# malani86/unet-DC-segmentation

Measured on AMD Instinct MI355X. Metric: images/sec fwd+bwd, 512x512x1 U-Net-DC, bs=8/GPU, higher is better.
Workload: dtype bf16

## Files before the change

### unet_dc_segmentation_amd/build.py

```python
from __future__ import annotations

import os
import shutil
import subprocess
import sys

HERE = os.path.dirname(os.path.abspath(__file__))
CSRC = os.path.join(HERE, "csrc")
SOURCES = ["abi.hip", "igemm_conv.hip", "igemm_dma.hip", "igemm_dma16.hip", "igemm_halo.hip", "igemm_lattice.hip", "wgrad.hip", "wgrad_dma.hip", "wgrad_fused.hip", "wgrad_rect.hip", "convt_wgrad.hip", "first_conv.hip", "first_conv_mfma.hip", "elementwise.hip", "loss.hip", "optim.hip", "ccl.hip", "preprocess.hip", "augment.hip", "density.hip"]
HEADERS = ["common.h", "kernels.h", "lds_dma.h", "wgrad_frag.h", "igemm_epilogue.h", "igemm_epilogue16.h", os.path.join("..", "..", "include", "unetdc_hip.h")]
OUT = os.path.join(HERE, "libunetdc_hip.so")


def _hipcc():
    for cand in (shutil.which("hipcc"), "/opt/rocm/bin/hipcc"):
        if cand and os.path.exists(cand):
            return cand
    raise RuntimeError("hipcc not found (ROCm toolchain required to build the gfx950 kernels)")


def needs_build():
    if not os.path.exists(OUT):
        return True
    t = os.path.getmtime(OUT)
    deps = [os.path.join(CSRC, f) for f in SOURCES + HEADERS]
    return any(os.path.getmtime(d) > t for d in deps)


FLAGS = ["--offload-arch=gfx950", "-O3", "-std=c++17", "-fPIC", "-Wall", "-Wno-unused-function", "-fno-slp-vectorize"]
OBJ_DIR = os.path.join(CSRC, "_obj")


def _includes(path, seen=None):
    import re
    seen = set() if seen is None else seen
    for m in re.finditer(r'^\s*#include\s+"([^"]+)"', open(path).read(), re.M):
        q = os.path.normpath(os.path.join(os.path.dirname(path), m.group(1)))
        if q not in seen and os.path.exists(q):
            seen.add(q)
            _includes(q, seen)
    return seen


def _object_key(src):
    import hashlib
    h = hashlib.sha256(" ".join(FLAGS).encode())
    for q in [src] + sorted(_includes(src)):
        h.update(open(q, "rb").read())
    return h.hexdigest()[:16]


def build(force=False, verbose=True):
    if not force and not needs_build():
        return OUT
    from concurrent.futures import ThreadPoolExecutor
    os.makedirs(OBJ_DIR, exist_ok=True)
    hipcc = _hipcc()

    def one(f):
        src = os.path.join(CSRC, f)
        obj = os.path.join(OBJ_DIR, f"{os.path.splitext(f)[0]}.{_object_key(src)}.o")
        if force or not os.path.exists(obj):
            for old in os.listdir(OBJ_DIR):
                if old.startswith(os.path.splitext(f)[0] + "."):
                    os.unlink(os.path.join(OBJ_DIR, old))
            cmd = [hipcc, *FLAGS, "-c", src, "-o", obj]
            if verbose:
                print("[unetdc build]", " ".join(cmd), flush=True)
            r = subprocess.run(cmd, capture_output=True, text=True)
            if r.returncode != 0:
                sys.stderr.write(r.stdout + r.stderr)
                raise RuntimeError(f"hipcc failed on {f}")
        return obj

    with ThreadPoolExecutor(max_workers=min(8, os.cpu_count() or 1)) as ex:
        objs = list(ex.map(one, SOURCES))
    cmd = [hipcc, "--offload-arch=gfx950", "-shared", "-fPIC", *objs, "-o", OUT]
    r = subprocess.run(cmd, capture_output=True, text=True)
    if r.returncode != 0:
        sys.stderr.write(r.stdout + r.stderr)
        raise RuntimeError("hipcc failed linking libunetdc_hip.so")
    return OUT


def _objdump():
    for cand in (shutil.which("llvm-objdump"), "/opt/rocm/lib/llvm/bin/llvm-objdump"):
        if cand and os.path.exists(cand):
            return cand
    raise RuntimeError("llvm-objdump not found")


def device_code_objects(so_path=OUT):
    import struct
    data = open(so_path, "rb").read()
    magic, pos, out = b"__CLANG_OFFLOAD_BUNDLE__", 0, []
    while True:
        i = data.find(magic, pos)
        if i < 0:
            return out
        n, = struct.unpack_from("<Q", data, i + 24)
        q = i + 32
        for _ in range(n):
            off, size, idl = struct.unpack_from("<QQQ", data, q)
            q += 24
            tid = data[q:q + idl].decode()
            q += idl
            if "gfx950" in tid and size:
                out.append(data[i + off:i + off + size])
        pos = i + 24


def packed_f32_report(so_path=OUT):
    import re
    import tempfile
    rep = {}
    for k, elf in enumerate(device_code_objects(so_path)):
        with tempfile.NamedTemporaryFile(suffix=".co") as f:
            f.write(elf)
            f.flush()
            r = subprocess.run([_objdump(), "-d", "--no-show-raw-insn", f.name], capture_output=True, text=True)
        if r.returncode != 0:
            raise RuntimeError("llvm-objdump failed: " + r.stderr[:300])
        cur = None
        for line in r.stdout.splitlines():
            m = re.match(r"^[0-9a-f]+ <(\S+)>:", line)
            if m:
                cur = m.group(1)
                rep.setdefault(cur, 0)
            elif cur and re.search(r"\bv_pk_(add|mul|fma)_f32\b", line):
                rep[cur] += 1
    return rep


if __name__ == "__main__":
    build(force="--force" in sys.argv)
```

### unet_dc_segmentation_amd/csrc/igemm_conv.hip

```cpp
#include <stdlib.h>

#include <stdio.h>

#include "kernels.h"

namespace unetdc {

template <typename T> struct Mma;
template <> struct Mma<bf16_t> {
  __device__ static __forceinline__ void run(f32x16& acc, const u32x4& a, const u32x4& b) {
    acc = __builtin_amdgcn_mfma_f32_32x32x16_bf16(__builtin_bit_cast(bf16x8, a), __builtin_bit_cast(bf16x8, b),
                                                  acc, 0, 0, 0);
  }
};
template <> struct Mma<float> {
  __device__ static __forceinline__ void run(f32x16& acc, const u32x4& a, const u32x4& b) {
#pragma unroll
    for (int s = 0; s < 4; ++s) {
      const unsigned int ua = a[s], ub = b[s];
      acc = __builtin_amdgcn_mfma_f32_32x32x2f32(bits_f32(ua), bits_f32(ub), acc, 0, 0, 0);
    }
  }
};

template <typename T> __device__ __forceinline__ void store_pair(T* dst, float v0, float v1);
template <> __device__ __forceinline__ void store_pair<float>(float* dst, float v0, float v1) {
  *reinterpret_cast<float2*>(dst) = make_float2(v0, v1);
}
template <> __device__ __forceinline__ void store_pair<bf16_t>(bf16_t* dst, float v0, float v1) {
  bf16_t lo = (bf16_t)v0, hi = (bf16_t)v1;
  *reinterpret_cast<unsigned int*>(dst) = (unsigned int)__builtin_bit_cast(unsigned short, lo) |
                                          ((unsigned int)__builtin_bit_cast(unsigned short, hi) << 16);
}

template <typename T, int WM, int WN>
__global__ __launch_bounds__(256, 2) void igemm_conv_kernel(const IgemmParams p) {
  constexpr int BM = 64 * WM, BN = 64 * WN;
  constexpr int AI = BM / 32, BI = BN / 32;
  constexpr int KE = 128 / (int)sizeof(T);
  constexpr int EPC = 16 / (int)sizeof(T);
  constexpr int STAGE = (BM + BN) * 128;
  extern __shared__ __attribute__((aligned(16))) unsigned char smem[];

  const int tid = threadIdx.x, lane = tid & 63, wave = tid >> 6;
  const int wm = wave / WN, wn = wave % WN;
  const int tile = xcd_remap(blockIdx.x, gridDim.x);
  const int mblk = tile / p.nblocks, nblk = tile - mblk * p.nblocks;
  const int m0 = mblk * BM, n0 = nblk * BN;
  const int c = tid & 7, r0 = tid >> 3;
  const T* __restrict__ xg = reinterpret_cast<const T*>(p.x);
  const T* __restrict__ wg = reinterpret_cast<const T*>(p.w);

  int pix[AI], ys[AI], xs[AI];
  unsigned tapmask = 0;
  const int HoWo = p.Ho * p.Wo;
#pragma unroll
  for (int i = 0; i < AI; ++i) {
    const int m = m0 + r0 + 32 * i;
    if (m < p.M) {
      const int n = m / HoWo, rem = m - n * HoWo;
      const int oy = rem / p.Wo, ox = rem - oy * p.Wo;
      ys[i] = oy * p.stride;
      xs[i] = ox * p.stride;
      pix[i] = (n * p.Hi + ys[i]) * p.Wi + xs[i];
    } else {
      ys[i] = -(1 << 28);
      xs[i] = 0;
      pix[i] = 0;
    }
    for (int t = 0; t < p.ntaps; ++t) {
      const int iy = ys[i] + p.offy[t], ix = xs[i] + p.offx[t];
      if ((unsigned)iy < (unsigned)p.Hi && (unsigned)ix < (unsigned)p.Wi) tapmask |= 1u << t;
    }
  }
  {
    unsigned* sm_u = reinterpret_cast<unsigned*>(smem);
    if (tid == 0) sm_u[0] = 0;
    __syncthreads();
    if (tapmask) atomicOr(&sm_u[0], tapmask);
    __syncthreads();
    tapmask = sm_u[0];
    __syncthreads();
  }
  const int nkc = p.Cin / KE;
  const int nsteps = __popc(tapmask) * nkc;

  const int swz_w = (r0 >> 1) & 7;
  int a_wr[AI], b_wr[BI];
#pragma unroll
  for (int i = 0; i < AI; ++i) a_wr[i] = (r0 + 32 * i) * 128 + ((c ^ swz_w) << 4);
#pragma unroll
  for (int i = 0; i < BI; ++i) {
    const int row = r0 + 32 * i, grp = row >> 6, cc = row & 63;
    const int lrow = grp * 64 + (cc & 1) * 32 + (cc >> 1);
    b_wr[i] = BM * 128 + lrow * 128 + ((c ^ ((lrow >> 1) & 7)) << 4);
  }
  const int r = lane & 31, h = lane >> 5;
  const int swz_r = (r >> 1) & 7;
  int a_rd[2][4], b_rd[2][4];
#pragma unroll
  for (int t2 = 0; t2 < 2; ++t2)
#pragma unroll
    for (int g = 0; g < 4; ++g) {
      const int ch = ((2 * g + h) ^ swz_r) << 4;
      a_rd[t2][g] = (wm * 64 + t2 * 32 + r) * 128 + ch;
      b_rd[t2][g] = BM * 128 + (wn * 64 + t2 * 32 + r) * 128 + ch;
    }

  f32x16 acc[2][2];
#pragma unroll
  for (int i = 0; i < 2; ++i)
#pragma unroll
    for (int j = 0; j < 2; ++j)
#pragma unroll
      for (int e = 0; e < 16; ++e) acc[i][j][e] = 0.f;

  u32x4 ra[AI], rb[BI];
  int lt = 0, lkc = 0;
  while (lt < p.ntaps && !((tapmask >> lt) & 1u)) ++lt;

  auto gload = [&]() {
    const int dy = p.offy[lt], dx = p.offx[lt];
    const int dpix = dy * p.Wi + dx;
    const int koff = lkc * KE + c * EPC;
#pragma unroll
    for (int i = 0; i < AI; ++i) {
      const int iy = ys[i] + dy, ix = xs[i] + dx;
      const bool ok = (unsigned)iy < (unsigned)p.Hi && (unsigned)ix < (unsigned)p.Wi;
      u32x4 v = {0u, 0u, 0u, 0u};
      if (ok) v = ld16(xg + ((long)(pix[i] + dpix) * p.ldx + koff));
      ra[i] = v;
    }
#pragma unroll
    for (int i = 0; i < BI; ++i)
      rb[i] = ld16(wg + ((long)(lt * p.Cout + n0 + r0 + 32 * i) * p.Cin + koff));
    if (++lkc == nkc) {
      lkc = 0;
      do { ++lt; } while (lt < p.ntaps && !((tapmask >> lt) & 1u));
    }
  };
  auto lds_store = [&](int stage) {
    unsigned char* base = smem + stage * STAGE;
#pragma unroll
    for (int i = 0; i < AI; ++i) st16(base + a_wr[i], ra[i]);
#pragma unroll
    for (int i = 0; i < BI; ++i) st16(base + b_wr[i], rb[i]);
  };

  if (nsteps > 0) {
    gload();
    lds_store(0);
  }
  __syncthreads();
  for (int s = 0; s < nsteps; ++s) {
    const bool more = (s + 1 < nsteps);
    if (more) gload();
    const unsigned char* base = smem + (s & 1) * STAGE;
#pragma unroll
    for (int g = 0; g < 4; ++g) {
      const u32x4 a0 = ld16(base + a_rd[0][g]), a1 = ld16(base + a_rd[1][g]);
      const u32x4 b0 = ld16(base + b_rd[0][g]), b1 = ld16(base + b_rd[1][g]);
      Mma<T>::run(acc[0][0], a0, b0);
      Mma<T>::run(acc[0][1], a0, b1);
      Mma<T>::run(acc[1][0], a1, b0);
      Mma<T>::run(acc[1][1], a1, b1);
    }
    if (more) lds_store((s + 1) & 1);
    __syncthreads();
  }

  const int col = n0 + wn * 64 + 2 * r;
  T* __restrict__ og = reinterpret_cast<T*>(p.out);
  float k0a = 0.f, k0b = 0.f, k1a = 0.f, k1b = 0.f;
  int shuf_ab = 0, shuf_co = col;
  if (p.mode == MODE_AFFINE_RELU) {
    k0a = p.scale[col]; k0b = p.scale[col + 1];
    k1a = p.shift[col]; k1b = p.shift[col + 1];
  } else if (p.mode == MODE_SHUFFLE) {
    shuf_ab = col / p.shuf_c;
    shuf_co = col - shuf_ab * p.shuf_c;
    if (p.bias) { k1a = p.bias[shuf_co]; k1b = p.bias[shuf_co + 1]; }
  } else if (p.bias) {
    k1a = p.bias[col]; k1b = p.bias[col + 1];
  }
  float s0 = 0.f, q0 = 0.f, s1 = 0.f, q1 = 0.f;
#pragma unroll
  for (int mi = 0; mi < 2; ++mi) {
#pragma unroll
    for (int reg = 0; reg < 16; ++reg) {
      const int m = m0 + wm * 64 + mi * 32 + (reg & 3) + 8 * (reg >> 2) + 4 * h;
      if (m >= p.M) continue;
      float v0 = acc[mi][0][reg], v1 = acc[mi][1][reg];
      if (p.mode == MODE_AFFINE_RELU) {
        v0 = fmaxf(fmaf(v0, k0a, k1a), 0.f);
        v1 = fmaxf(fmaf(v1, k0b, k1b), 0.f);
        store_pair<T>(og + (long)m * p.ldo + col, v0, v1);
      } else if (p.mode == MODE_SHUFFLE) {
        v0 += k1a; v1 += k1b;
        const int n = m / HoWo, rem = m - n * HoWo;
        const int oy = rem / p.Wo, ox = rem - oy * p.Wo;
        const long dst = ((long)(n * 2 * p.Ho + 2 * oy + (shuf_ab >> 1)) * (2 * p.Wo) + 2 * ox + (shuf_ab & 1));
        store_pair<T>(og + dst * p.ldo + shuf_co, v0, v1);
      } else {
        v0 += k1a; v1 += k1b;
        store_pair<T>(og + (long)m * p.ldo + col, v0, v1);
        if (p.mode == MODE_STATS) {
          const float t0 = round_through<T>(v0), t1 = round_through<T>(v1);
          s0 += t0; q0 = fmaf(t0, t0, q0);
          s1 += t1; q1 = fmaf(t1, t1, q1);
        }
      }
    }
  }
  if (p.mode == MODE_STATS) {
    s0 += __shfl_xor(s0, 32, 64); q0 += __shfl_xor(q0, 32, 64);
    s1 += __shfl_xor(s1, 32, 64); q1 += __shfl_xor(q1, 32, 64);
    float* red = reinterpret_cast<float*>(smem);
    if (h == 0) {
      red[(wave * 4 + 0) * 32 + r] = s0;
      red[(wave * 4 + 1) * 32 + r] = q0;
      red[(wave * 4 + 2) * 32 + r] = s1;
      red[(wave * 4 + 3) * 32 + r] = q1;
    }
    __syncthreads();
    if (tid < BN) {
      const int wn2 = tid >> 6, c2 = tid & 63, r2 = c2 >> 1, e = c2 & 1;
      float su = 0.f, sq = 0.f;
#pragma unroll
      for (int w2 = 0; w2 < WM; ++w2) {
        su += red[((w2 * WN + wn2) * 4 + e * 2 + 0) * 32 + r2];
        sq += red[((w2 * WN + wn2) * 4 + e * 2 + 1) * 32 + r2];
      }
      p.stats[((long)mblk * 2 + 0) * p.Cout + n0 + tid] = su;
      p.stats[((long)mblk * 2 + 1) * p.Cout + n0 + tid] = sq;
    }
  }
}

int igemm_mblocks(long M, int Cout) { (void)Cout; return ceil_div(M, 256); }

template <typename T, int WM, int WN>
static int launch_cfg(IgemmParams& p, hipStream_t stream) {
  constexpr int BM = 64 * WM, BN = 64 * WN;
  constexpr int LDS = 2 * (BM + BN) * 128;
  if (const int rc_ = ensure_dynamic_lds(reinterpret_cast<const void*>(&igemm_conv_kernel<T, WM, WN>), LDS, "igemm_conv_kernel")) return rc_;
  p.mblocks = ceil_div(p.M, BM);
  p.nblocks = p.Cout / BN;
  const long nwg = (long)p.mblocks * p.nblocks;
  hipLaunchKernelGGL((igemm_conv_kernel<T, WM, WN>), dim3((unsigned)nwg), dim3(256), LDS, stream, p);
  char nm[96];
  snprintf(nm, sizeof(nm), "igemm_conv_kernel<%s, %d, %d>", sizeof(T) == 2 ? "__bf16" : "float", WM, WN);
  note_kernel(nm);
  return check_launch("igemm_conv_kernel");
}

IgemmPlan plan_igemm(const IgemmParams& p, int dtype) {
  IgemmPlan pl{};
  const bool lattice = igemm_lattice_supported(p, dtype);
  if (p.in_scale) {
    if (lattice && p.mode == MODE_STATS && (p.Cout % 128 == 0 || p.Cin <= 256)) {
      pl.route = IGEMM_LATTICE;
      pl.writes_act = p.Cout % 128 == 0 && (long)p.M * p.Cin * 2 < (1L << 32);
    }
    return pl;
  }
  if (lattice) {
    pl.route = IGEMM_LATTICE;
    return pl;
  }
  if (igemm_halo_supported(p, dtype)) {
    pl.route = IGEMM_HALO;
    return pl;
  }
  const long es = dtype == UNETDC_BF16 ? 2 : 4;
  const long HoWo = (long)p.Ho * p.Wo;
  const long xbytes = (p.M / HoWo) * p.Hi * p.Wi * p.ldx * es;
  const long wbytes = (long)p.ntaps * p.Cout * p.Cin * es;
  const long opix = p.mode == MODE_SHUFFLE ? 4L * p.M : (long)p.M;
  const long obytes = opix * p.ldo * es, ybytes = p.mode == MODE_BNBWD ? (long)p.M * p.bn_ldy * es : 0;
  if (!(xbytes < (1L << 31) && wbytes < (1L << 31) && obytes < (1L << 32) && ybytes < (1L << 32) && p.M % HoWo == 0)) {
    pl.route = IGEMM_FIRSTGEN;
    pl.cfg = (p.Cout % 128 == 0) && p.mode != MODE_STATS;
    return pl;
  }
  const long blocks_a = (long)((p.M + 255) / 256) * (p.Cout / 256);
  const bool use_a = p.Cout % 256 == 0 && p.M >= 256 * 64 && blocks_a >= 200;
  const bool use_b = !use_a && p.Cout % 128 == 0;
  pl.route = IGEMM_DMA;
  pl.cfg = use_a ? 1 : (use_b ? 2 : 3);
  if (dtype == UNETDC_BF16 && p.M % 16 == 0 && !(p.mode == MODE_SHUFFLE && p.Wo % 16 != 0)) {
    pl.route = IGEMM_DMA16;
    const long blocks_b = (long)((p.M + 255) / 256) * (p.Cout / 128);
    if (pl.cfg == 2 && p.mode == MODE_SHUFFLE && p.Cout % 256 == 0 && blocks_a >= 200) pl.cfg = 1;
    else if (pl.cfg == 2 && blocks_b >= 100 && blocks_b < 200) pl.cfg = 3;
  }
  return pl;
}

int launch_igemm(IgemmParams& p, int dtype, hipStream_t stream) {
  const int esz = dtype == UNETDC_BF16 ? 2 : 4;
  const int ke = 128 / esz;
  UNETDC_REQUIRE(dtype == UNETDC_F32 || dtype == UNETDC_BF16, "igemm: bad dtype %d", dtype);
  UNETDC_REQUIRE(p.x && p.w && p.out, "igemm: null tensor pointer");
  UNETDC_REQUIRE(p.M > 0 && p.Cin > 0 && p.Cout > 0, "igemm: empty problem");
  UNETDC_REQUIRE(p.Cin % ke == 0, "igemm: Cin=%d must be a multiple of %d for this dtype", p.Cin, ke);
  UNETDC_REQUIRE(p.Cout % 64 == 0, "igemm: Cout=%d must be a multiple of 64", p.Cout);
  UNETDC_REQUIRE(p.ldx % (16 / esz) == 0 && p.ldo % (16 / esz) == 0, "igemm: ld not 16-byte aligned");
  UNETDC_REQUIRE(((uintptr_t)p.x % 16 == 0) && ((uintptr_t)p.w % 16 == 0) && ((uintptr_t)p.out % 16 == 0),
                 "igemm: pointers must be 16-byte aligned");
  UNETDC_REQUIRE(p.ntaps >= 1 && p.ntaps <= 9, "igemm: ntaps out of range");
  UNETDC_REQUIRE((long)p.M < (1L << 31) - 512, "igemm: too many pixels");
  if (p.mode == MODE_SHUFFLE) UNETDC_REQUIRE(p.shuf_c % 64 == 0, "igemm: convT channels must be a multiple of 64");
  if (p.mode == MODE_STATS) UNETDC_REQUIRE(p.stats != nullptr, "igemm: stats buffer missing");
  if (p.mode == MODE_AFFINE_RELU) UNETDC_REQUIRE(p.scale && p.shift, "igemm: scale/shift missing");
  if (p.mode == MODE_BNBWD)
    UNETDC_REQUIRE(p.stats && p.bn_y && p.scale && p.shift && p.bn_mean && p.bn_rstd, "igemm: BN-backward inputs missing");
  {
    const long howo = (long)p.Ho * p.Wo;
    const bool p2 = (p.Wo & (p.Wo - 1)) == 0 && (howo & (howo - 1)) == 0;
    p.wo_shift = p2 ? __builtin_ctz((unsigned)p.Wo) : -1;
    p.howo_shift = p2 ? __builtin_ctzl((unsigned long)howo) : -1;
  }
  const IgemmPlan pl = plan_igemm(p, dtype);
  switch (pl.route) {
    case IGEMM_LATTICE: return launch_igemm_lattice(p, stream);
    case IGEMM_HALO: return launch_igemm_halo(p, dtype, stream);
    case IGEMM_DMA: return launch_igemm_dma(p, pl.cfg, dtype, stream);
    case IGEMM_DMA16: return launch_igemm_dma16(p, pl.cfg, stream);
    case IGEMM_FIRSTGEN:
      if (p.mode == MODE_BNBWD) {
        set_error("igemm: the first-generation kernel has no fused BatchNorm-backward sums");
        return UNETDC_EUNSUPPORTED;
      }
      if (dtype == UNETDC_BF16) return pl.cfg ? launch_cfg<bf16_t, 2, 2>(p, stream) : launch_cfg<bf16_t, 4, 1>(p, stream);
      return pl.cfg ? launch_cfg<float, 2, 2>(p, stream) : launch_cfg<float, 4, 1>(p, stream);
  }
  set_error("igemm: input normalisation asked for a shape / configuration the lattice kernel does not take");
  return UNETDC_EUNSUPPORTED;
}

}
```

### unet_dc_segmentation_amd/csrc/kernels.h

```cpp
#pragma once
#include "common.h"
#include "../../include/unetdc_hip.h"

namespace unetdc {

enum { MODE_STORE = 0, MODE_STATS = 1, MODE_AFFINE_RELU = 2, MODE_SHUFFLE = 3, MODE_BNBWD = 4 };
#define UNETDC_EUNSUPPORTED (-4)

struct IgemmParams {
  const void* x;
  const void* w;
  void* out;
  const float* bias;
  const float* scale;
  const float* shift;
  float* stats;
  const void* bn_y;
  const float* bn_mean;
  const float* bn_rstd;
  int bn_ldy;
  int M, Ho, Wo, Hi, Wi, Cin, Cout, ldx, ldo, ntaps, stride, mode, shuf_c;
  int mblocks, nblocks;
  int wo_shift, howo_shift;
  int quad_bpr, quad_bpi;
  const float* in_scale;
  const float* in_shift;
  void* act_out;
  int ld_act;
  int offy[9];
  int offx[9];
};
enum IgemmRoute {
  IGEMM_UNSUPPORTED = 0,
  IGEMM_LATTICE,
  IGEMM_HALO,
  IGEMM_DMA,
  IGEMM_DMA16,
  IGEMM_FIRSTGEN,
};
struct IgemmPlan {
  int route;
  int cfg;
  bool writes_act;
};
IgemmPlan plan_igemm(const IgemmParams& p, int dtype);
int launch_igemm(IgemmParams& p, int dtype, hipStream_t stream);
int igemm_mblocks(long M, int Cout);
bool igemm_lattice_supported(const IgemmParams& p, int dtype);
bool igemm_halo_supported(const IgemmParams& p, int dtype);
int launch_igemm_lattice(IgemmParams& p, hipStream_t stream);
int launch_igemm_halo(IgemmParams& p, int dtype, hipStream_t stream);
int launch_igemm_dma(IgemmParams& p, int cfg, int dtype, hipStream_t stream);
int launch_igemm_dma16(IgemmParams& p, int cfg, hipStream_t stream);

struct WgradParams {
  const void* a;
  const void* b;
  float* part;
  int N, H, W, Hb, Wb, CI, CJ, lda, ldb, ntaps, stride;
  int P;
  int chunk;
  int ksplit, itiles, jtiles;
  int adv_y, adv_x;
  int offy[9];
  int offx[9];
  const float* in_scale;
  const float* in_shift;
};
enum WgradRoute {
  WGRAD_UNSUPPORTED = 0,
  WGRAD_CONVT,
  WGRAD_RECT,
  WGRAD_FUSED,
  WGRAD_DMA,
  WGRAD_LEGACY,
};
struct WgradPlan {
  int route;
  int ksplit;
  int chunk, tw, step;
  int steps_per_half;
  long workspace;
};
WgradPlan plan_wgrad(const WgradParams& p, int dtype);
long wgrad_workspace_bound(int N, int H, int W, int CI, int CJ, int ntaps, int dtype);
int launch_wgrad(WgradParams& p, float* out, void* workspace, long workspace_bytes, int dtype, hipStream_t stream);
bool convt_wgrad_split(int N, int H, int W, int CI, int CJ, int& ksplit, int& steps_per_half);
int launch_convt_wgrad_fused(const WgradParams& w, const WgradPlan& pl, hipStream_t stream);
int wgrad_rect_units(int N, int H, int W, int CI, int CJ, int d);
int launch_wgrad_rect(const WgradParams& w, const WgradPlan& pl, float* out, hipStream_t stream);
bool wgrad_fused_supported(int N, int H, int W, int CI, int CJ, int lda, int ldb, int d, int ntaps, int stride, int dtype);
bool wgrad_fused_bnin_supported(int d, int dtype);
long wgrad_fused_workspace_bytes(int N, int H, int W, int CI, int CJ, int dtype);
int launch_wgrad_fused(const WgradParams& w, int dtype, int* units_out, hipStream_t stream);
int wgrad_dma_tile(int CI, int CJ);
int wgrad_dma_pixel_step(int dtype, int tw);
int launch_wgrad_dma_kernel(WgradParams& p, int tw, int dtype, hipStream_t stream);

struct FirstParams {
  const float* x;
  const float* w;
  const float* bias;
  const float* scale;
  const float* shift;
  void* y;
  float* stats;
  int N, H, W, Cin, Cout, ldy, dil;
};
struct FirstWgradParams {
  const float* x;
  const void* dy;
  float* part;
  int N, H, W, Cin, Cout, lddy, dil;
  const void* bn_y; int bn_ldy;
  const float* bn_scale; const float* bn_shift; const float* bn_mean; const float* bn_rstd; const float* bn_k;
};
struct FirstPlan {
  bool mfma;
  int fwd_blocks;
  bool wgrad_mfma;
  int wgrad_blocks;
  int rows_blocks;
  long workspace;
};
FirstPlan plan_first(long P, int Cin, int Cout);
int launch_first_fwd(FirstParams& p, int dtype, hipStream_t stream);
bool first_wgrad_bn_supported(int N, int H, int W, int Cin, int Cout, int dil, int dtype);
int launch_bn_bwd_coeffs(const float* pre_parts, int pre_nparts, long count, const float* gamma, const float* rstd, float* dgamma,
                         float* dbeta, float* dbias, float* coeffs, int C, hipStream_t stream);
int first_mfma_mblocks(long P);
int first_mfma_wgrad_blocks(long P);
int launch_first_mfma_fwd(FirstParams& p, int blocks, int dtype, hipStream_t stream);
int launch_first_mfma_wgrad(FirstWgradParams& p, int blocks, int dtype, hipStream_t stream);
int launch_first_wgrad(FirstWgradParams& p, float* dw, void* workspace, long workspace_bytes, int dtype,
                       hipStream_t stream);
int launch_first_dgrad(const void* dy, int lddy, const float* w, float* dx, int N, int H, int W, int Cin, int Cout, int dil,
                       int dtype, hipStream_t stream);

struct ApplyParams {
  const void* y; void* a; void* pooled;
  const float* scale; const float* shift;
  int N, H, W, C, ldy, lda, ldp;
};
struct BnBwdParams {
  const void* dskip; const void* dpool; const void* y; void* dy;
  const float* scale; const float* shift; const float* mean; const float* rstd;
  const float* k1; const float* k2; const float* k3;
  float* parts;
  int N, H, W, C, lds, ldp, ldy, lddy;
  const float* head_dprobs; const float* head_probs; const float* head_w;
};
struct HeadParams {
  const void* a; const float* w; const float* b; float* probs;
  const float* dprobs; void* da; float* parts;
  int N, H, W, C, OC, lda, ldda;
  const void* bn_y; const float* bn_scale; const float* bn_shift; const float* bn_mean; const float* bn_rstd;
  float* bn_parts;
  int bn_ldy;
};
int launch_bn_finalize(const float* parts, int nparts, long count, const float* gamma, const float* beta, float eps,
                       float momentum, float* rm, float* rv, float* scale, float* shift, float* mean, float* rstd,
                       int C, hipStream_t stream);
int launch_bn_eval_affine(const float* gamma, const float* beta, const float* rm, const float* rv,
                          const float* conv_bias, float eps, float* scale, float* shift, int C, hipStream_t stream);
int launch_apply(ApplyParams& p, int dtype, hipStream_t stream);
long bn_bwd_workspace_bytes(int N, int H, int W, int C, int pooled, int dtype);
int launch_bn_bwd(BnBwdParams& p, const float* gamma, float* dgamma, float* dbeta, float* dbias, void* workspace,
                  long workspace_bytes, const float* pre_parts, int pre_nparts, int dtype, hipStream_t stream,
                  bool frozen = false);
int launch_bn_frozen_affine(const float* gamma, const float* beta, const float* rm, const float* rv, float eps, float* scale,
                            float* shift, float* mean, float* rstd, int C, hipStream_t stream);
int launch_stats_colsum_rows(const float* parts, int nparts, int row_floats, int c0, int c, float* out, hipStream_t stream);
int launch_bn_bwd_reduce_only(BnBwdParams& p, float* parts, long parts_floats, int* nparts, int dtype,
                              hipStream_t stream);
long head_bwd_workspace_bytes(int N, int H, int W, int C, int OC, int dtype);
int launch_head_fwd(HeadParams& p, int dtype, hipStream_t stream);
int launch_head_bwd(HeadParams& p, float* dw, float* db, void* workspace, long workspace_bytes, int dtype,
                    hipStream_t stream, int* bn_nparts = nullptr, long bn_parts_floats = 0);
int launch_pack_conv3x3(const float* w, void* wf, void* wd, int Co, int Ci, int dtype, hipStream_t stream);
int launch_pack_convT2x2(const float* w, void* wf, void* wd, int Ci, int Co, int dtype, hipStream_t stream);
int launch_pack_many(const void* table_dev, int n, long total, int dtype, hipStream_t stream);
int launch_adam_step(const void* table_dev, int n, long total_blocks, const float* flat_grad, double lr, double beta1,
                     double beta2, double eps, long step, double grad_scale, int dtype, hipStream_t stream);
int launch_stats_colsum(const float* parts, int nparts, int ctotal, int c0, int c, float* out, hipStream_t stream);
long channel_sum_workspace_bytes(long P, int C);
int launch_channel_sum(const void* x, int ldx, float* out, void* workspace, long workspace_bytes, long P, int C,
                       int dtype, hipStream_t stream);

int launch_mask_from_probs(const float* probs, int ph, int pw, float thresh, unsigned char* mask, int oh, int ow,
                           hipStream_t stream);
int launch_mask_from_probs_linear(const float* probs, int ph, int pw, float thresh, unsigned char* mask, int oh, int ow,
                                  const int* xofs, const short* xcoef, const int* yofs, const short* ycoef, hipStream_t stream);
long ccl_workspace_bytes(int h, int w);
int launch_ccl_stats(const unsigned char* mask, int h, int w, int min_area, void* workspace, long workspace_bytes,
                     int* out_count, int* out_area, long long* out_sumy, long long* out_sumx, int* out_root, int max_out,
                     hipStream_t stream);

constexpr int AUG_HFLIP = 1, AUG_VFLIP = 2, AUG_BC = 4;
constexpr int AUG_MAX_SEEDS = 64;
constexpr int AUG_MAX_BATCH = 32;
struct AugRecord {
  int src, flags, k, field;
  float alpha, beta_max;
  int reserved[2];
};
long elastic_fields_workspace_bytes(int n, int h, int w, double sigma);
int launch_elastic_fields(const unsigned* seeds, int n, int h, int w, double sigma, float alpha, float* fields,
                          void* workspace, long workspace_bytes, hipStream_t stream);
int launch_augment_gather(const float* cache_img, const unsigned char* cache_mask, int ncache, int c, int h, int w,
                          const AugRecord* params, int n, const float* fields, int nfields, float* out_img, float* out_mask,
                          hipStream_t stream);

long rolling_ball_workspace_bytes(int h, int w, int cn);
int launch_rolling_ball(const unsigned char* src, unsigned char* dst, int h, int w, int cn, int k, void* workspace,
                        long workspace_bytes, hipStream_t stream);
int launch_resize_linear_chw(const unsigned char* src, int h, int w, int cn, float* dst, int dh, int dw, const int* xofs,
                             const short* xa, const int* yofs, const short* ya, hipStream_t stream);
int launch_morph_rect(const unsigned char* src, unsigned char* dst, int h, int w, int k, bool is_max, hipStream_t stream);

long density_workspace_bytes(int h, int w);
int launch_density_maps(const unsigned char* rgb, const unsigned char* mask, int h, int w, const int* dcount, const int* darea,
                        const long long* dsumy, const long long* dsumx, int dcap, int nb_layers, double sigma,
                        const double* taps, void* workspace, long workspace_bytes, unetdc_density_stats* stats,
                        unsigned char* radial_index, unsigned char* spatial_index, unsigned char* out_blur,
                        unsigned char* out_roi, unsigned char* out_ring, float* out_radial, float* out_spatial,
                        hipStream_t stream);
int launch_density_sqrt(const long long* x, double* out, long n, hipStream_t stream);

long loss_workspace_bytes(int nimg, long hw);
int launch_loss_fwd(const float* p, const float* t, float* loss_out, float* coef, void* workspace, long workspace_bytes,
                    int nimg, long hw, float alpha, float gamma, float ratio, float smooth, hipStream_t stream);
int launch_loss_bwd(const float* p, const float* t, const float* coef, const float* gout, float* dp, int nimg, long hw,
                    float alpha, float gamma, float ratio, hipStream_t stream);

}
```

Baseline: 761.7.

## Add dedicated register-resident-weight kernel for bf16 transposed-conv forward

```diff
diff --git a/unet_dc_segmentation_amd/build.py b/unet_dc_segmentation_amd/build.py
--- a/unet_dc_segmentation_amd/build.py
+++ b/unet_dc_segmentation_amd/build.py
@@ -7,7 +7,7 @@
 
 HERE = os.path.dirname(os.path.abspath(__file__))
 CSRC = os.path.join(HERE, "csrc")
-SOURCES = ["abi.hip", "igemm_conv.hip", "igemm_dma.hip", "igemm_dma16.hip", "igemm_halo.hip", "igemm_lattice.hip", "wgrad.hip", "wgrad_dma.hip", "wgrad_fused.hip", "wgrad_rect.hip", "convt_wgrad.hip", "first_conv.hip", "first_conv_mfma.hip", "elementwise.hip", "loss.hip", "optim.hip", "ccl.hip", "preprocess.hip", "augment.hip", "density.hip"]
+SOURCES = ["abi.hip", "igemm_conv.hip", "igemm_dma.hip", "igemm_dma16.hip", "igemm_halo.hip", "igemm_lattice.hip", "wgrad.hip", "wgrad_dma.hip", "wgrad_fused.hip", "wgrad_rect.hip", "convt_wgrad.hip", "convt_fwd.hip", "first_conv.hip", "first_conv_mfma.hip", "elementwise.hip", "loss.hip", "optim.hip", "ccl.hip", "preprocess.hip", "augment.hip", "density.hip"]
 HEADERS = ["common.h", "kernels.h", "lds_dma.h", "wgrad_frag.h", "igemm_epilogue.h", "igemm_epilogue16.h", os.path.join("..", "..", "include", "unetdc_hip.h")]
 OUT = os.path.join(HERE, "libunetdc_hip.so")
 
diff --git a/unet_dc_segmentation_amd/csrc/convt_fwd.hip b/unet_dc_segmentation_amd/csrc/convt_fwd.hip
--- /dev/null
+++ b/unet_dc_segmentation_amd/csrc/convt_fwd.hip
@@ -0,0 +1,186 @@
+#include <stdio.h>
+#include <stdlib.h>
+
+#include "igemm_epilogue16.h"
+#include "kernels.h"
+#include "lds_dma.h"
+
+namespace unetdc {
+
+struct ConvtFwdParams {
+  const void* x;
+  const void* w;
+  const float* bias;
+  void* up;
+  int M, H, W, Cout, ldx, ldup;
+  int w_shift, hw_shift;
+  int mtiles, nblocks;
+};
+
+constexpr unsigned CONVT_OOB = 0x80000000u;
+
+template <int CIN> struct ConvtFwdCfg {
+  static constexpr int WGS = 2;
+  static constexpr int LDS = 2 * 64 * CIN * 2 + 256 * 4;
+};
+
+template <int CIN>
+__global__ __launch_bounds__(256, ConvtFwdCfg<CIN>::WGS) void convt_fwd_kernel(const ConvtFwdParams p) {
+#if defined(__HIP_DEVICE_COMPILE__)
+  constexpr int NKC = CIN / 64;
+  constexpr int NKG = CIN / 32;
+  constexpr int BM = 64;
+  constexpr int TMT = BM / 16;
+  constexpr int STAGE = BM * CIN * 2;
+  constexpr int PER = BM * NKC / 32;
+  constexpr int NST = TMT * 2;
+  static_assert(CIN == 128 || CIN == 256, "K");
+  static_assert(NST <= 63, "vmcnt is a 6-bit counter");
+  extern __shared__ __attribute__((aligned(16))) unsigned char smem[];
+
+  const int tid = threadIdx.x, lane = tid & 63;
+  const int wave = __builtin_amdgcn_readfirstlane(tid >> 6);
+  const int bid = xcd_remap(blockIdx.x, gridDim.x);
+  const int nblk = bid % p.nblocks;
+  const int mstride = gridDim.x / p.nblocks;
+  int mt = bid / p.nblocks;
+  if (mt >= p.mtiles) return;
+  const unsigned lds_base = lds_addr_of(smem);
+
+  const unsigned xbytes = (unsigned)p.M * (unsigned)p.ldx * 2u;
+  const unsigned obytes = (unsigned)p.M * 4u * (unsigned)p.ldup * 2u;
+  const __amdgpu_buffer_rsrc_t xr = __builtin_amdgcn_make_buffer_rsrc(const_cast<void*>(p.x), 0, xbytes, 0x00020000);
+  const __amdgpu_buffer_rsrc_t orr = __builtin_amdgcn_make_buffer_rsrc(p.up, 0, obytes, 0x00020000);
+
+  const int sub = lane >> 3, pc = lane & 7;
+  const int drow = wave * 8 + sub;
+  const unsigned dchunk = (unsigned)((pc ^ ((drow >> 1) & 7)) << 4);
+  auto issue = [&](int stage, int tile) {
+    const int m0 = tile * BM;
+    const unsigned sbase = lds_base + (unsigned)__builtin_amdgcn_readfirstlane(stage) * STAGE;
+#pragma unroll
+    for (int j = 0; j < PER; ++j) {
+      const int row = drow + 32 * (j & 1), kc = j >> 1;
+      const int m = m0 + row;
+      lds_dma16(xr, sbase + (wave + 4 * j) * 1024, m < p.M ? (unsigned)m * (unsigned)p.ldx * 2u + (unsigned)(kc * 128) + dchunk
+                                                             : CONVT_OOB, 0u);
+    }
+  };
+  issue(0, mt);
+
+  const int c16 = lane & 15, rb = lane >> 4;
+  const int nw = nblk * 256 + wave * 64;
+  const int ab = nw / p.Cout, ch = nw - ab * p.Cout + 8 * rb;
+  u32x4 wf[4][NKG];
+#pragma unroll
+  for (int j = 0; j < 4; ++j) {
+    const int col = nw + 32 * (j >> 1) + 8 * (c16 >> 2) + 4 * (j & 1) + (c16 & 3);
+    const u32x4* src = reinterpret_cast<const u32x4*>(static_cast<const bf16_t*>(p.w) + (long)col * CIN + 8 * rb);
+#pragma unroll
+    for (int g = 0; g < NKG; ++g) wf[j][g] = src[4 * g];
+  }
+  float* bias_l = reinterpret_cast<float*>(smem + 2 * STAGE);
+  bias_l[tid] = p.bias ? p.bias[(nblk * 256 + tid) % p.Cout] : 0.f;
+  const float* bias_w = bias_l + wave * 64 + 8 * rb;
+
+  const int swz = (c16 >> 1) & 7;
+  int x_rd[2];
+#pragma unroll
+  for (int h = 0; h < 2; ++h) x_rd[h] = c16 * 128 + (((4 * h + rb) ^ swz) << 4);
+  const int H2 = 2 * p.H, W2 = 2 * p.W, HW = p.H * p.W;
+  const unsigned ldob = (unsigned)p.ldup * 2u;
+
+  int cur = 0;
+  for (bool first = true;; first = false) {
+    if (first) wait_vmcnt<0>(); else wait_vmcnt<NST>();
+    raw_barrier();
+    const int next = mt + mstride;
+    const bool more = next < p.mtiles;
+    if (more) issue(cur ^ 1, next);
+
+    f32x4 acc[TMT][4];
+#pragma unroll
+    for (int i = 0; i < TMT; ++i)
+#pragma unroll
+      for (int j = 0; j < 4; ++j)
+#pragma unroll
+        for (int e = 0; e < 4; ++e) acc[i][j][e] = 0.f;
+    const unsigned char* base = smem + cur * STAGE;
+#pragma unroll
+    for (int g = 0; g < NKG; ++g)
+#pragma unroll
+      for (int i = 0; i < TMT; ++i) {
+        const u32x4 xf = ld16(base + (g >> 1) * BM * 128 + i * 16 * 128 + x_rd[g & 1]);
+#pragma unroll
+        for (int j = 0; j < 4; ++j)
+          acc[i][j] = __builtin_amdgcn_mfma_f32_16x16x32_bf16(__builtin_bit_cast(bf16x8, wf[j][g]), __builtin_bit_cast(bf16x8, xf),
+                                                              acc[i][j], 0, 0, 0);
+      }
+
+    const int m0 = mt * BM;
+#pragma unroll
+    for (int i = 0; i < TMT; ++i) {
+      const int m = m0 + 16 * i + c16;
+      int n, y, xx;
+      if (p.w_shift >= 0) {
+        n = m >> p.hw_shift;
+        const int rem = m & (HW - 1);
+        y = rem >> p.w_shift;
+        xx = rem & (p.W - 1);
+      } else {
+        n = m / HW;
+        const int rem = m - n * HW;
+        y = rem / p.W;
+        xx = rem - y * p.W;
+      }
+      const unsigned opix = (unsigned)((n * H2 + 2 * y + (ab >> 1)) * W2 + 2 * xx + (ab & 1));
+      const unsigned voff = m < p.M ? opix * ldob + (unsigned)ch * 2u : CONVT_OOB;
+#pragma unroll
+      for (int q = 0; q < 2; ++q) {
+        const f32x4 lo = acc[i][2 * q], hi = acc[i][2 * q + 1];
+        const f32x4 bl = *reinterpret_cast<const f32x4*>(bias_w + 32 * q), bh = *reinterpret_cast<const f32x4*>(bias_w + 32 * q + 4);
+        const u32x2 a = pack4_bf16(lo[0] + bl[0], lo[1] + bl[1], lo[2] + bl[2], lo[3] + bl[3]);
+        const u32x2 b = pack4_bf16(hi[0] + bh[0], hi[1] + bh[1], hi[2] + bh[2], hi[3] + bh[3]);
+        const u32x4 v = {a[0], a[1], b[0], b[1]};
+        __builtin_amdgcn_raw_buffer_store_b128(v, orr, voff, (unsigned)q * 64u, 0);
+      }
+    }
+    if (!more) break;
+    mt = next;
+    cur ^= 1;
+  }
+#endif
+}
+
+template <int CIN>
+static int launch_cfg(const ConvtFwdParams& q, hipStream_t stream) {
+  constexpr int LDS = ConvtFwdCfg<CIN>::LDS;
+  const void* fn = reinterpret_cast<const void*>(&convt_fwd_kernel<CIN>);
+  if (const int rc = ensure_dynamic_lds(fn, LDS, "convt_fwd_kernel")) return rc;
+  const long items = (long)q.mtiles * q.nblocks;
+  constexpr int FULL = 256 * ConvtFwdCfg<CIN>::WGS;
+  const long nwg = items < FULL ? items : FULL - FULL % q.nblocks;
+  hipLaunchKernelGGL((convt_fwd_kernel<CIN>), dim3((unsigned)nwg), dim3(256), LDS, stream, q);
+  note_kernel(CIN == 128 ? "convt_fwd_kernel<128>" : "convt_fwd_kernel<256>");
+  return check_launch("convt_fwd_kernel");
+}
+
+bool convt_fwd_supported(const IgemmParams& p, int dtype) {
+  if (dtype != UNETDC_BF16 || p.mode != MODE_SHUFFLE || p.ntaps != 1 || p.stride != 1) return false;
+  if (!(p.Cin == 128 || p.Cin == 256) || p.shuf_c % 64 != 0 || p.Cout != 4 * p.shuf_c || p.Cout % 256 != 0) return false;
+  return (long)p.M * p.ldx * 2 < (1L << 31) && 4L * p.M * p.ldo * 2 < (1L << 31);
+}
+
+int launch_convt_fwd(IgemmParams& p, hipStream_t stream) {
+  UNETDC_REQUIRE(convt_fwd_supported(p, UNETDC_BF16), "convt_fwd: unsupported shape");
+  ConvtFwdParams q{};
+  q.x = p.x; q.w = p.w; q.bias = p.bias; q.up = p.out;
+  q.M = p.M; q.H = p.Ho; q.W = p.Wo; q.Cout = p.shuf_c; q.ldx = p.ldx; q.ldup = p.ldo;
+  q.w_shift = p.wo_shift; q.hw_shift = p.howo_shift;
+  q.mtiles = ceil_div(p.M, 64);
+  q.nblocks = p.Cout / 256;
+  p.mblocks = q.mtiles; p.nblocks = q.nblocks;
+  return p.Cin == 128 ? launch_cfg<128>(q, stream) : launch_cfg<256>(q, stream);
+}
+
+}
diff --git a/unet_dc_segmentation_amd/csrc/igemm_conv.hip b/unet_dc_segmentation_amd/csrc/igemm_conv.hip
--- a/unet_dc_segmentation_amd/csrc/igemm_conv.hip
+++ b/unet_dc_segmentation_amd/csrc/igemm_conv.hip
@@ -293,6 +293,7 @@
     const long blocks_b = (long)((p.M + 255) / 256) * (p.Cout / 128);
     if (pl.cfg == 2 && p.mode == MODE_SHUFFLE && p.Cout % 256 == 0 && blocks_a >= 200) pl.cfg = 1;
     else if (pl.cfg == 2 && blocks_b >= 100 && blocks_b < 200) pl.cfg = 3;
+    if (convt_fwd_supported(p, dtype)) pl.route = IGEMM_CONVT_FWD;
   }
   return pl;
 }
@@ -327,6 +328,7 @@
     case IGEMM_HALO: return launch_igemm_halo(p, dtype, stream);
     case IGEMM_DMA: return launch_igemm_dma(p, pl.cfg, dtype, stream);
     case IGEMM_DMA16: return launch_igemm_dma16(p, pl.cfg, stream);
+    case IGEMM_CONVT_FWD: return launch_convt_fwd(p, stream);
     case IGEMM_FIRSTGEN:
       if (p.mode == MODE_BNBWD) {
         set_error("igemm: the first-generation kernel has no fused BatchNorm-backward sums");
diff --git a/unet_dc_segmentation_amd/csrc/kernels.h b/unet_dc_segmentation_amd/csrc/kernels.h
--- a/unet_dc_segmentation_amd/csrc/kernels.h
+++ b/unet_dc_segmentation_amd/csrc/kernels.h
@@ -37,6 +37,7 @@
   IGEMM_DMA,
   IGEMM_DMA16,
   IGEMM_FIRSTGEN,
+  IGEMM_CONVT_FWD,
 };
 struct IgemmPlan {
   int route;
@@ -52,6 +53,8 @@
 int launch_igemm_halo(IgemmParams& p, int dtype, hipStream_t stream);
 int launch_igemm_dma(IgemmParams& p, int cfg, int dtype, hipStream_t stream);
 int launch_igemm_dma16(IgemmParams& p, int cfg, hipStream_t stream);
+bool convt_fwd_supported(const IgemmParams& p, int dtype);
+int launch_convt_fwd(IgemmParams& p, hipStream_t stream);
 
 struct WgradParams {
   const void* a;
```

After: 764.1 (median of 6 runs). No clear change (+0.3%).
